# MetaHG/mitsuba2

Hardware: AMD Instinct MI355X
Metric: Msample/s, cbox 1024x1024@256spp per GPU, path integrator (max_depth=-1, rr_depth=5) (higher is better)
Workload: dtype f32

## Files before the change

mitsuba2_amd/csrc/device_scene.h:

```cpp
#pragma once
#include "device_math.h"
#include "device_bsdf.h"
#include "device_envmap.h"
#include "flat_worklist.h"

namespace mtsamd {

constexpr uint32_t kLeafFlag = 0x80000000u;
constexpr uint32_t kLeafCountShift = 27;
constexpr uint32_t kLeafStartMask = (1u << kLeafCountShift) - 1u;
constexpr uint32_t kNoPrim = 0xffffffffu;

#ifndef MTS_BVH4
#define MTS_BVH4 1
#endif
#if MTS_BVH4
typedef uint2 StackEntry;
typedef uint64_t StackRaw;
#else
typedef uint32_t StackEntry;
typedef uint32_t StackRaw;
#endif


// ... 20 lines not shown
    const float4 *nodes;
    const uint4 *qnodes;
    const uint4 *wnodes;
    uint32_t wroot, n_wnodes;
    float q_lo[3], q_step[3], q_inv_step[3];
    const float4 *tris;
    uint32_t root;
    uint32_t n_nodes, n_slots, n_prims;
    uint32_t lds_nodes;
    uint32_t lds_slots;
    uint32_t stack_depth;
    uint32_t walk_lds_depth, walk_blocks;
    StackEntry *walk_spill;
    const float *tri_pos;
    const float *tri_nrm;
    const float *tri_uv;
    const uint32_t *prim_shape;
    const DevShape *shapes;
    const DevBsdf *bsdfs;
    const DevEmitter *emitters; uint32_t n_emitters;
    uint32_t n_shapes, n_bsdfs;
    const DevTexture *textures; uint32_t n_textures;
    const float *area_pmf, *area_cdf;
    const float4 *flat_recs;
    const float4 *flat_pairs;
    uint32_t flat, n_pairs, n_clusters;
    int32_t env_emitter;
    const DevEnvmap *envmap;
    uint32_t general;
};
constexpr uint32_t kFlatMaxPrims = 64;

struct LdsView {
    const float4 *nodes;
    const float4 *tris;
    uint32_t *stack;
    uint32_t stride;
    StackEntry *spill;
    uint32_t spill_stride, stack_lds_depth;
    const float4 *flat;
    const float4 *pairs;
    const float4 *clusters;
    const DevShape *shapes;
    const DevBsdf *bsdfs;
    const DevEmitter *emitters;
    const float *pmf, *cdf;
    uint32_t *wl;
};

#ifndef MTS_FLAT_WORKLIST
#define MTS_FLAT_WORKLIST 1
#endif
#ifndef MTS_FLAT_WL_ROUNDS
#define MTS_FLAT_WL_ROUNDS 5
#endif
constexpr uint32_t kWlItems = 64u * MTS_FLAT_WL_ROUNDS;
constexpr uint32_t kWlWords = 128u + kWlItems / 2u;

inline uint32_t flat_shape_count(const SceneView &sv) { return sv.n_shapes; }

template <bool FLAT>
MTS_DEV LdsView lds_stage(const SceneView &sv, float4 *smem) {
    LdsView l = {};
    l.stride = blockDim.x;
    if (FLAT) {
        float4 *f = smem;
        for (uint32_t i = threadIdx.x; i < 4u * sv.n_prims; i += blockDim.x) f[i] = sv.flat_recs[i];
        l.flat = f;
        float4 *pr = f + 4u * sv.n_prims;
        for (uint32_t i = threadIdx.x; i < 5u * sv.n_pairs; i += blockDim.x) pr[i] = sv.flat_pairs[i];
        if (threadIdx.x < 5u) pr[5u * sv.n_pairs + threadIdx.x] = make_float4(0.0f, 0.0f, 0.0f, 0.0f);
        l.pairs = pr;
        float4 *cl = pr + 5u * sv.n_pairs + 5u;
        for (uint32_t i = threadIdx.x; i < 2u * sv.n_clusters; i += blockDim.x) cl[i] = sv.flat_pairs[5u * sv.n_pairs + i];
        l.clusters = cl;
        uint32_t *w = reinterpret_cast<uint32_t *>(cl + 2u * sv.n_clusters);
        const uint32_t n_sh = (sizeof(DevShape) / 4u) * sv.n_shapes, n_bs = (sizeof(DevBsdf) / 4u) * sv.n_bsdfs,
                       n_em = (sizeof(DevEmitter) / 4u) * sv.n_emitters;
        const uint32_t *g_sh = reinterpret_cast<const uint32_t *>(sv.shapes), *g_bs = reinterpret_cast<const uint32_t *>(sv.bsdfs),
                       *g_em = reinterpret_cast<const uint32_t *>(sv.emitters);
        for (uint32_t i = threadIdx.x; i < n_sh; i += blockDim.x) w[i] = g_sh[i];
        l.shapes = reinterpret_cast<const DevShape *>(w); w += n_sh;
        for (uint32_t i = threadIdx.x; i < n_bs; i += blockDim.x) w[i] = g_bs[i];
        l.bsdfs = reinterpret_cast<const DevBsdf *>(w); w += n_bs;
        for (uint32_t i = threadIdx.x; i < n_em; i += blockDim.x) w[i] = g_em[i];
        l.emitters = reinterpret_cast<const DevEmitter *>(w); w += n_em;
        float *fw = reinterpret_cast<float *>(w);
        for (uint32_t i = threadIdx.x; i < sv.n_prims; i += blockDim.x) { fw[i] = sv.area_pmf[i]; fw[sv.n_prims + i] = sv.area_cdf[i]; }
        l.pmf = fw; l.cdf = fw + sv.n_prims;
        const uint32_t wl_off = (uint32_t) (reinterpret_cast<uint32_t *>(fw + 2u * sv.n_prims) - reinterpret_cast<uint32_t *>(smem));
        l.wl = MTS_FLAT_WORKLIST ? reinterpret_cast<uint32_t *>(smem) + ((wl_off + 1u) & ~1u) : nullptr;
    } else {
        float4 *n = smem;
        float4 *t = n + 4u * sv.lds_nodes;
        for (uint32_t i = threadIdx.x; i < 4u * sv.lds_nodes; i += blockDim.x) n[i] = sv.nodes[i];
        for (uint32_t i = threadIdx.x; i < 3u * sv.lds_slots; i += blockDim.x) t[i] = sv.tris[i];
        l.nodes = n; l.tris = t;
        l.stack = reinterpret_cast<uint32_t *>(t + 3u * sv.lds_slots);
    }
    __syncthreads();
    return l;
}
inline size_t lds_bytes(const SceneView &sv, uint32_t block) {
    if (sv.flat)
        return (size_t) 64 * sv.n_prims + (size_t) 80 * (sv.n_pairs + 1) + (size_t) 32 * sv.n_clusters + sizeof(DevShape) * sv.n_shapes + sizeof(DevBsdf) * sv.n_bsdfs +
               sizeof(DevEmitter) * sv.n_emitters + (size_t) 8 * sv.n_prims +
               (MTS_FLAT_WORKLIST ? 4u + (size_t) 4 * kWlWords * (block / 64u) : 0u);
// ... 570 lines not shown
    bool any = false;
    if (!(MTS_CULL_STATS & 2)) tri_tests += sv.n_prims;
    const v2f ox = splat(o.x), oy = splat(o.y), oz = splat(o.z), dx = splat(d.x), dy = splat(d.y), dz = splat(d.z);
    const f3 inv = mk3(clamp_inv(d.x), clamp_inv(d.y), clamp_inv(d.z));
    const float4 *rec = lds.pairs;
    for (uint32_t c = 0; c < sv.n_clusters; ++c) {
        const float4 lo = lds.clusters[2u * c], hi = lds.clusters[2u * c + 1u];
        const uint32_t n = __float_as_uint(lo.w);
        const float ax = (lo.x - o.x) * inv.x, bx = (hi.x - o.x) * inv.x;
        const float ay = (lo.y - o.y) * inv.y, by = (hi.y - o.y) * inv.y;
        const float az = (lo.z - o.z) * inv.z, bz = (hi.z - o.z) * inv.z;
        const float tn = fmaxf(fmaxf(fminf(ax, bx), fminf(ay, by)), fmaxf(fminf(az, bz), mint));
        const float tf = fminf(fminf(fmaxf(ax, bx), fmaxf(ay, by)), fminf(fmaxf(az, bz), maxt));
        if (__ballot(!any && tn <= tf) == 0ull) { rec += 5u * n; continue; }
        if (MTS_CULL_STATS & 2) tri_tests += 2u * n;
        for (uint32_t i = 0; i < n; ++i) {
            const float4 q0 = rec[0], q1 = rec[1], q2 = rec[2], q3 = rec[3], q4 = rec[4];
            rec += 5;
            const PairUvt r = pair_test(q0, q1, q2, q3, q4, ox, oy, oz, dx, dy, dz);
            const bool ok_a = tri_accept(r.u.x, r.v.x, r.uv.x, r.t.x, mint, maxt);
            const bool ok_b = tri_accept(r.u.y, r.v.y, r.uv.y, r.t.y, mint, maxt);
            any = any || ok_a || ok_b;
        }
    }
    return any;
}

static_assert(kFlatMaxPrims <= 64u, "a pair mask is 32 bits");
template <bool ANY>
MTS_DEV bool traverse_flat_worklist(const SceneView &sv, const LdsView &lds, f3 o, f3 d, float mint, float maxt, Hit &hit, uint32_t &tri_tests) {
    const uint64_t active = __ballot(1);
    const uint32_t n_act = (uint32_t) __popcll(active), lane = lane_id(), rank = mask_rank(active);
    const f3 inv = mk3(clamp_inv(d.x), clamp_inv(d.y), clamp_inv(d.z));
    uint32_t pairs = 0u, first = 0u;
    for (uint32_t c = 0; c < sv.n_clusters; ++c) {
        const float4 lo = lds.clusters[2u * c], hi = lds.clusters[2u * c + 1u];
        const uint32_t n = __float_as_uint(lo.w);
        const float ax = (lo.x - o.x) * inv.x, bx = (hi.x - o.x) * inv.x;
        const float ay = (lo.y - o.y) * inv.y, by = (hi.y - o.y) * inv.y;
        const float az = (lo.z - o.z) * inv.z, bz = (hi.z - o.z) * inv.z;
        const float tn = fmaxf(fmaxf(fminf(ax, bx), fminf(ay, by)), fmaxf(fminf(az, bz), mint));
        const float tf = fminf(fminf(fmaxf(ax, bx), fmaxf(ay, by)), fminf(fmaxf(az, bz), maxt));
        const uint32_t bits = (uint32_t) ((1ull << n) - 1ull) << first;
        pairs |= tn <= tf ? bits : 0u;
        first += n;
    }
    const uint32_t cnt = (uint32_t) __popc(pairs);
    uint32_t pos = 0u, total = 0u;
#pragma unroll
    for (uint32_t b = 0; b < 6u; ++b) {
        const uint64_t m = __ballot((cnt >> b) & 1u);
        pos += mask_rank(m) << b; total += (uint32_t) __popcll(m) << b;
    }
    if (total > kWlItems || total > MTS_FLAT_WL_ROUNDS * n_act) return traverse_flat<ANY>(sv, lds, o, d, mint, maxt, hit, tri_tests);
    constexpr bool kRealCount = (MTS_CULL_STATS & (ANY ? 2 : 1)) != 0;
    if (!kRealCount) tri_tests += sv.n_prims;
    uint32_t *ws = lds.wl + (threadIdx.x >> 6) * kWlWords;
    unsigned long long *key = reinterpret_cast<unsigned long long *>(ws);
    uint16_t *tbl = reinterpret_cast<uint16_t *>(ws + 128u);
    if (ANY) ws[lane] = 0u;
    else key[lane] = kWlNoKey;
    wl_push_items(tbl, pos, pairs, lane);
    __builtin_amdgcn_fence(__ATOMIC_RELEASE, "wavefront");
    __builtin_amdgcn_wave_barrier();
    __builtin_amdgcn_fence(__ATOMIC_ACQUIRE, "wavefront");
    for (uint32_t j0 = 0u; j0 < total; j0 += n_act) {
        const uint32_t j = j0 + rank;
        const uint32_t item = j < total ? (uint32_t) tbl[j] : wl_item(lane, sv.n_pairs);
        const uint32_t owner = wl_item_owner(item), pair = wl_item_pair(item);
        const int addr = (int) (owner << 2);
        const float rox = __int_as_float(__builtin_amdgcn_ds_bpermute(addr, __float_as_int(o.x)));
        const float roy = __int_as_float(__builtin_amdgcn_ds_bpermute(addr, __float_as_int(o.y)));
        const float roz = __int_as_float(__builtin_amdgcn_ds_bpermute(addr, __float_as_int(o.z)));
        const float rdx = __int_as_float(__builtin_amdgcn_ds_bpermute(addr, __float_as_int(d.x)));
        const float rdy = __int_as_float(__builtin_amdgcn_ds_bpermute(addr, __float_as_int(d.y)));
        const float rdz = __int_as_float(__builtin_amdgcn_ds_bpermute(addr, __float_as_int(d.z)));
        const float rmint = __int_as_float(__builtin_amdgcn_ds_bpermute(addr, __float_as_int(mint)));
        const float rmaxt = __int_as_float(__builtin_amdgcn_ds_bpermute(addr, __float_as_int(maxt)));
        const float4 *rec = lds.pairs + 5u * pair;
        const float4 q0 = rec[0], q1 = rec[1], q2 = rec[2], q3 = rec[3], q4 = rec[4];
        const PairUvt r = pair_test(q0, q1, q2, q3, q4, splat(rox), splat(roy), splat(roz), splat(rdx), splat(rdy), splat(rdz));
        const bool ok_a = tri_accept(r.u.x, r.v.x, r.uv.x, r.t.x, rmint, rmaxt);
        const bool ok_b = tri_accept(r.u.y, r.v.y, r.uv.y, r.t.y, rmint, rmaxt);
        if (kRealCount && j < total) tri_tests += 2u;
        if (ANY) {
            if (ok_a || ok_b) ws[owner] = 1u;
        } else if (ok_a || ok_b) {
            const uint64_t ka = ok_a ? wl_key(r.t.x, 2u * pair) : kWlNoKey, kb = ok_b ? wl_key(r.t.y, 2u * pair + 1u) : kWlNoKey;
            atomicMin(&key[owner], (unsigned long long) (ka < kb ? ka : kb));
        }
        if (ANY) {
            __builtin_amdgcn_fence(__ATOMIC_RELEASE, "wavefront");
            __builtin_amdgcn_wave_barrier();
            __builtin_amdgcn_fence(__ATOMIC_ACQUIRE, "wavefront");
            if (__ballot(ws[lane] == 0u && pos + cnt > j0 + n_act) == 0ull) break;
        }
    }
    __builtin_amdgcn_fence(__ATOMIC_RELEASE, "wavefront");
    __builtin_amdgcn_wave_barrier();
    __builtin_amdgcn_fence(__ATOMIC_ACQUIRE, "wavefront");
    if (ANY) return ws[lane] != 0u;
    const uint64_t k = key[lane];
    hit.t = maxt; hit.prim = kNoPrim; hit.u = 0.0f; hit.v = 0.0f;
    if (k == kWlNoKey) return false;
    hit.prim = wl_key_prim(k);
    hit.t = flat_hit_uv(lds, o, d, hit.prim, hit.u, hit.v);
    return true;
// ... 345 lines not shown
```

mitsuba2_amd/csrc/kernels.h:

```cpp
#pragma once
#include <hip/hip_runtime.h>
#include "device_scene.h"
#include "device_spectral.h"

namespace mtsamd {

struct PoolView {
    float4 *ray_o, *ray_d, *thr, *res;
    uint4 *rng;
    uint2 *misc;
    float *xi;
    float2 *aux;
    float4 *hit, *sh_o, *sh_d, *nee;
    uint32_t *sh_slot;
};

struct RowMap { int32_t row0, local_rows, tile_rows, part, count; };
MTS_DEV int32_t row_to_global(const RowMap &m, int32_t lr) {
    if (m.count <= 1) return m.row0 + lr;
    int32_t t = lr / m.tile_rows;
    return (t * m.count + m.part) * m.tile_rows + (lr - t * m.tile_rows);
}
MTS_DEV int32_t row_to_local(const RowMap &m, int32_t gr) {
    if (m.count <= 1) { int32_t lr = gr - m.row0; return (lr >= 0 && lr < m.local_rows) ? lr : -1; }
// ... 48 lines not shown
    if (k >= chains) return n;
    const uint32_t lo = ((uint32_t) ((uint64_t) n * k / chains) + kChainAlign - 1u) & ~(kChainAlign - 1u);
    return lo < n ? lo : n;
}
__host__ __device__ inline uint32_t chunk_owner(uint32_t wave, uint32_t n, uint32_t chains) {
    if (chains <= 1u) return wave;
    uint32_t s_min = n, k = 0u, lo_k = 0u, extra_before = 0u;
    for (uint32_t c = 0; c < chains; ++c) {
        const uint32_t lo = chain_first(c, n, chains), hi = chain_first(c + 1u, n, chains);
        s_min = hi - lo < s_min ? hi - lo : s_min;
        if (wave >= lo && wave < hi) { k = c; lo_k = lo; }
    }
    const uint32_t i = wave - lo_k;
    if (i < s_min) return i * chains + k;
    for (uint32_t c = 0; c < k; ++c) extra_before += chain_first(c + 1u, n, chains) - chain_first(c, n, chains) - s_min;
    return s_min * chains + extra_before + (i - s_min);
}

struct FilmParams {
    const float4 *out_rgba;
    const float2 *out_pos;
    float *film;
    FilterView filter;
    uint64_t first_ordinal, n_samples;
    uint32_t plane_pix0, plane_pixels;
    RowMap rows;
    int32_t spp, crop_x, crop_y, crop_w, crop_h;
    int32_t row0, row1;
    int32_t pass_lr0, pass_rows, tiles_x, tiles_y;
    int32_t tile_h;
    int32_t slices;
    float *partials;
};

struct AdjointParams {
    RenderParams rp;
    FilterView filter;
    uint64_t n_samples;
    const float *dimage;
    const float *film;
    float *grad_bsdf;
    float *grad_tex;
    float *grad_emitter;
    float *grad_env;
    int32_t pg_bsdf; DevBsdf pg_plus, pg_minus; float pg_inv_2h; float *grad_param;
};

struct RayStreams {
    const float *ox, *oy, *oz, *dx, *dy, *dz, *mint, *maxt;
    const uint8_t *active;
};

size_t bounce_lds_bytes(const SceneView &sv);
hipError_t launch_bounce(const RenderParams &p, hipStream_t s);
hipError_t launch_split_stage(const RenderParams &p, int stage, hipStream_t s);
uint32_t trace_lds_depth(const SceneView &sv);
uint32_t trace_top_nodes(const SceneView &sv);
uint32_t trace_group();
size_t trace_spill_words(const SceneView &sv, uint32_t n_waves);
hipError_t launch_direct(const RenderParams &p, uint64_t n, hipStream_t s);
hipError_t launch_adjoint(const AdjointParams &a, hipStream_t s);
hipError_t launch_adjoint_env(const AdjointParams &a, hipStream_t s);
hipError_t launch_adjoint_param(const AdjointParams &a, hipStream_t s);
hipError_t launch_finish(const RenderParams &p, uint64_t alive, hipStream_t s);
hipError_t launch_mega(const RenderParams &p, hipStream_t s);
hipError_t upload_spectral_tables(const float *x, const float *y, const float *z, const float *d65);
hipError_t launch_film_gather(const FilmParams &p, hipStream_t s);
hipError_t launch_film_tiles(const FilmParams &p, hipStream_t s);
bool film_tiles_supported(const FilterView &f);
void film_tile_grid(FilmParams &p);
size_t film_partial_floats(const FilmParams &p);
hipError_t launch_ray_intersect(const SceneView &sv, uint64_t n, const RayStreams &r, int mode, float *t,
                                uint32_t *prim, uint32_t *shape, float *u, float *v, float *si26,
                                hipStream_t s);
hipError_t launch_ray_test(const SceneView &sv, uint64_t n, const RayStreams &r, uint8_t *hit, hipStream_t s);
hipError_t launch_camera_rays(const CameraView &cam, uint64_t n, const float *sx, const float *sy, const float *apx, const float *apy, float *ox,
                              float *oy, float *oz, float *dx, float *dy, float *dz, float *mint, float *maxt,
                              hipStream_t s);
hipError_t launch_imageblock_put(const FilterView &f, int32_t w, int32_t h, int32_t ox, int32_t oy, int32_t ch,
                                 int32_t border, uint64_t n, const float *pos, const float *values, float *data,
                                 hipStream_t s);
hipError_t launch_put_block(const float *src, int32_t sw, int32_t sh, int32_t sox, int32_t soy, int32_t sb,
                            float *dst, int32_t dw, int32_t dh, int32_t dox, int32_t doy, int32_t db, int32_t ch,
                            hipStream_t s);
hipError_t launch_square_stream(float4 *rgba, uint64_t n, hipStream_t s);
hipError_t launch_moment_pack(const float *values5, const float *squares5, float *film11, uint64_t n_pixels, hipStream_t s);
hipError_t launch_roughplastic_tables(DevBsdf *bsdfs, uint32_t index, float *table, const float *gl, int res_t, int res_r, hipStream_t s);
hipError_t launch_film_develop(const float *xyzaw, uint64_t n, float *rgba, hipStream_t s);
hipError_t launch_libm_eval(int fn, uint64_t n, const float *x, const float *y, float *out, hipStream_t s);

}
```

mitsuba2_amd/csrc/kernels.hip:

```cpp
#include "kernels.h"

namespace mtsamd {

constexpr int kBlock = 256;

struct PathState {
    f3 o, d; float mint, maxt;
    f3 thr; float bs_pdf;
    f3 res; float eta;
    Pcg32 rng;
    uint32_t ordinal, depth, flags;
};

template <bool NT = false>
MTS_DEV void load_state(const PoolView &p, size_t i, PathState &s) {
    float4 a = ld_stream<NT>(p.ray_o + i), b = ld_stream<NT>(p.ray_d + i), c = ld_stream<NT>(p.thr + i), e = ld_stream<NT>(p.res + i);
    uint4 r = ld_stream<NT>(p.rng + i); uint2 m = ld_stream<NT>(p.misc + i);
    s.o = mk3(a.x, a.y, a.z); s.mint = a.w;
    s.d = mk3(b.x, b.y, b.z); s.maxt = b.w;
    s.thr = mk3(c.x, c.y, c.z); s.bs_pdf = c.w;
    s.res = mk3(e.x, e.y, e.z); s.eta = e.w;
    s.rng.state = (uint64_t) r.x | ((uint64_t) r.y << 32);
    s.rng.inc = (uint64_t) r.z | ((uint64_t) r.w << 32);
    s.ordinal = m.x; s.depth = m.y & 0xffffu; s.flags = m.y >> 16;
}
template <bool NT = false>
MTS_DEV void store_state(const PoolView &p, size_t i, const PathState &s) {
    st_stream<NT>(p.ray_o + i, make_float4(s.o.x, s.o.y, s.o.z, s.mint));
    st_stream<NT>(p.ray_d + i, make_float4(s.d.x, s.d.y, s.d.z, s.maxt));
    st_stream<NT>(p.thr + i, make_float4(s.thr.x, s.thr.y, s.thr.z, s.bs_pdf));
    p.res[i] = make_float4(s.res.x, s.res.y, s.res.z, s.eta);
    st_stream<NT>(p.rng + i, make_uint4((uint32_t) s.rng.state, (uint32_t) (s.rng.state >> 32), (uint32_t) s.rng.inc,
                                        (uint32_t) (s.rng.inc >> 32)));
    st_stream<NT>(p.misc + i, make_uint2(s.ordinal, (s.depth & 0xffffu) | (s.flags << 16)));
}

struct Counters { uint32_t closest, any, segments, tri_tests; };

struct VertexRec {
    f3 E, Nc, Tp, rho; float invq;
    f3 T; int32_t rr_channel;
    uint32_t texel; f2 w1; int32_t bsdf; uint32_t has_bsdf;
    float ew, nk; int32_t em_hit, em_nee;
};

struct Deferred {
    Hit hit; bool found;
    bool pending; f3 so, sd; float smint, smaxt; float nee[4];
};

constexpr uint32_t kFlagDelta = 4u;

struct EnvGradCtx { f3 delta; float *grad; };
MTS_DEV void env_grad_add(const DevEnvmap &e, float u, float v, f3 coeff, const EnvGradCtx &eg) {
    u *= (float) (e.w - 1); v *= (float) (e.h - 1);
    const uint32_t px = min((uint32_t) u, (uint32_t) (e.w - 2)), py = min((uint32_t) v, (uint32_t) (e.h - 2));
    const float w1x = u - (float) px, w1y = v - (float) py, w0x = 1.0f - w1x, w0y = 1.0f - w1y;
// ... 778 lines not shown
#pragma unroll
    for (int k = 0; k < 4; ++k)
        for (int off = 32; off > 0; off >>= 1) tot[k] += __shfl_xor(tot[k], off);
    if (lane_id() == 0) {
        unsigned long long *ws = reinterpret_cast<unsigned long long *>(P.wave_stats + 4u * (size_t) ((gid >> 6) % P.n_waves));
        for (int k = 0; k < 4; ++k) if (tot[k]) atomicAdd(ws + k, (unsigned long long) tot[k]);
    }
}

hipError_t launch_direct(const RenderParams &p, uint64_t n, hipStream_t s) {
    const uint32_t blocks = (uint32_t) ((n + kBlock - 1) / kBlock);
    const size_t lds = bounce_lds_bytes(p.sv);
    if (p.sv.general == 2u) {
        if (p.sv.flat) hipLaunchKernelGGL((k_direct<true, true, true>), dim3(blocks), dim3(kBlock), lds, s, p, n);
        else hipLaunchKernelGGL((k_direct<false, true, true>), dim3(blocks), dim3(kBlock), lds, s, p, n);
    } else if (p.sv.general) {
        if (p.sv.flat) hipLaunchKernelGGL((k_direct<true, true>), dim3(blocks), dim3(kBlock), lds, s, p, n);
        else hipLaunchKernelGGL((k_direct<false, true>), dim3(blocks), dim3(kBlock), lds, s, p, n);
    } else {
        if (p.sv.flat) hipLaunchKernelGGL((k_direct<true, false>), dim3(blocks), dim3(kBlock), lds, s, p, n);
        else hipLaunchKernelGGL((k_direct<false, false>), dim3(blocks), dim3(kBlock), lds, s, p, n);
    }
    return hipGetLastError();
}

constexpr uint32_t kFlagZombie = 2u;

template <bool GENERAL, bool FLAT>
MTS_DEV bool step_deferred(const RenderParams &P, const LdsView &lds, PathState &s, Counters &c, Deferred &df) {
    return bounce_step<FLAT, false, FLAT ? 2 : 1, GENERAL>(P, lds, s, c, nullptr, &df);
}
template <bool GENERAL, bool FLAT>
MTS_DEV bool step_deferred(const RenderParams &P, const LdsView &lds, PathStateS &s, Counters &c, Deferred &df) {
    return bounce_step_spectral<FLAT, FLAT ? 2 : 1, GENERAL>(P, lds, s, c, &df);
}
MTS_DEV void add_nee(PathState &s, const float (&nee)[4]) { s.res = mk3(s.res.x + nee[0], s.res.y + nee[1], s.res.z + nee[2]); }
MTS_DEV void add_nee(PathStateS &s, const float (&nee)[4]) {
#pragma unroll
    for (int k = 0; k < kWav; ++k) s.res.v[k] += nee[k];
}
MTS_DEV void finish_path(const RenderParams &P, const PathState &s) { store_result(P, s); }
MTS_DEV void finish_path(const RenderParams &P, const PathStateS &s) { store_result_spectral(P, s); }
MTS_DEV void start_path(const RenderParams &P, uint64_t ordinal, uint32_t lp, uint32_t j, PathState &s) { generate_path(P, ordinal, lp, j, s); }
MTS_DEV void start_path(const RenderParams &P, uint64_t ordinal, uint32_t lp, uint32_t j, PathStateS &s) { generate_path_spectral(P, ordinal, lp, j, s); }

#ifndef MTS_SHADE_WAVES_MIN
#define MTS_SHADE_WAVES_MIN 4
#endif
#ifndef MTS_SHADE_WAVES_MIN_RGB_DIFFUSE
#define MTS_SHADE_WAVES_MIN_RGB_DIFFUSE 5
#endif
template <typename State, bool GENERAL> struct ShadeWaves { static constexpr int kMin = MTS_SHADE_WAVES_MIN; };
template <> struct ShadeWaves<PathState, false> { static constexpr int kMin = MTS_SHADE_WAVES_MIN_RGB_DIFFUSE; };
constexpr uint32_t kShadowRing = 128u;
template <typename State> struct ShadowRing { float4 *o, *d, *nee; uint32_t *slot; };

template <typename State, bool GENERAL>
MTS_DEV void drain_shadow_ring(const RenderParams &P, const LdsView &lds, const ShadowRing<State> &q, uint32_t head, uint32_t count,
                               size_t base, Counters &c) {
    __builtin_amdgcn_fence(__ATOMIC_SEQ_CST, "workgroup");
    const uint32_t lane = lane_id();
    if (lane < count) {
        const uint32_t k = (head + lane) & (kShadowRing - 1u);
        const float4 o = q.o[k], d = q.d[k];
        Hit h;
        if (!traverse<true, true>(P.sv, lds, mk3(o.x, o.y, o.z), mk3(d.x, d.y, d.z), o.w, d.w, h, c.tri_tests)) {
            const size_t slot = base + q.slot[k];
            float4 r = P.out.res[slot];
            const float4 e = q.nee[k];
            r.x += e.x; r.y += e.y; r.z += e.z; r.w += e.w;
            P.out.res[slot] = r;
        }
    }
}

#ifndef MTS_NT_STREAMS
#define MTS_NT_STREAMS 3
#endif
#ifndef MTS_PRIMARY_SHADOW
#define MTS_PRIMARY_SHADOW 1
#endif
#ifndef MTS_SURV_ORDER
#define MTS_SURV_ORDER 1
#endif
template <typename State, bool GENERAL, bool FLAT, bool INLINE = false>
__global__ __launch_bounds__(kBlock) __attribute__((amdgpu_waves_per_eu(FLAT ? MTS_BOUNCE_WAVES : ShadeWaves<State, GENERAL>::kMin, FLAT ? MTS_BOUNCE_WAVES : 8)))
void k_shade(const RenderParams P) {
    static_assert(FLAT || !INLINE, "the in-kernel shadow queue is for LDS-resident scenes");
    constexpr bool kNT = !FLAT && (MTS_NT_STREAMS & 2) != 0;
    extern __shared__ float4 smem[];
    LdsView lds = {};
    const uint32_t gw = (FLAT && P.gather_w > 4u) ? P.gather_w : 4u;
    const uint32_t hw = threadIdx.x >> 6;
    const uint32_t wave = gw > 4u ? P.wave_first + blockIdx.x * gw + hw : P.wave_first + ((blockIdx.x * kBlock + threadIdx.x) >> 6);
    const uint32_t wave_last = P.wave_last ? P.wave_last : P.n_waves;
    __shared__ uint32_t s_cnt[kBlock / 64u], s_surv[kBlock / 64u];
    __shared__ uint32_t s_pre[FLAT ? 1025 : 1];
    if (FLAT && gw > 4u) {
        const uint32_t g0 = wave - hw;
        for (uint32_t k = threadIdx.x; k < gw; k += kBlock) s_pre[k + 1u] = (g0 + k < wave_last) ? P.count_in[g0 + k] : 0u;
        if (threadIdx.x == 0u) s_pre[0] = 0u;
        __syncthreads();
        if (hw == 0u) {
            const uint32_t per = (gw + 63u) / 64u, ln = lane_id();
            uint32_t local = 0u;
            for (uint32_t i = 0; i < per; ++i) { const uint32_t idx = ln * per + i; if (idx < gw) local += s_pre[idx + 1u]; }
            uint32_t incl = local;
            for (uint32_t off = 1u; off < 64u; off <<= 1) { const uint32_t v = __shfl_up(incl, off); if (ln >= off) incl += v; }
            uint32_t run = incl - local;
            for (uint32_t i = 0; i < per; ++i) { const uint32_t idx = ln * per + i; if (idx < gw) { run += s_pre[idx + 1u]; s_pre[idx + 1u] = run; } }
        }
        __syncthreads();
        if (s_pre[gw] == 0u) {
            for (uint32_t k = threadIdx.x; k < gw; k += kBlock) if (g0 + k < wave_last) P.count_out[g0 + k] = 0u;
            return;
        }
        lds = lds_stage<true>(P.sv, smem);
    } else if (FLAT) {
        const uint32_t n_own = wave < wave_last ? P.count_in[wave] : 0u;
        if (lane_id() == 0u) { s_cnt[threadIdx.x >> 6] = n_own; s_surv[threadIdx.x >> 6] = (wave < wave_last && MTS_SURV_ORDER) ? min(P.count_in[P.n_waves + wave], n_own) : 0u; }
        const bool work = wave < wave_last && (n_own > 0u || P.cursor[wave] < P.cursor_end[wave]);
        if (!__syncthreads_or(work ? 1 : 0)) {
            if (wave < wave_last && lane_id() == 0u) {
                P.count_out[wave] = 0u;
                if (!INLINE) P.count_shadow[wave] = 0u;
            }
            return;
        }
        lds = lds_stage<true>(P.sv, smem);
    }
    ShadowRing<State> ring = {};
    if (INLINE) {
        float4 *qb = smem + P.lds_queue_offset + (size_t) (threadIdx.x >> 6) * (kShadowRing * 13u / 4u);
        ring.o = qb; ring.d = qb + kShadowRing; ring.nee = qb + 2u * kShadowRing;
        ring.slot = reinterpret_cast<uint32_t *>(qb + 3u * kShadowRing);
    }
    if (wave >= wave_last) return;
    const uint32_t lane = lane_id();
    const size_t base = (size_t) wave * P.seg_cap;
    uint32_t n_out = 0;
    Counters c = { 0u, 0u, 0u, 0u };
    uint32_t n_sh = 0;
    uint32_t q_head = 0, q_count = 0;
    const uint32_t wg_wave0 = wave - (threadIdx.x >> 6);
    const uint32_t n_valid = FLAT ? min((uint32_t) (kBlock / 64u), wave_last - wg_wave0) : 1u;
    uint32_t reg[2u * (kBlock / 64u)], surv4[kBlock / 64u], n_in = 0;
    if (FLAT && gw > 4u) {
        n_in = s_pre[gw];
    } else if (FLAT) {
#pragma unroll
        for (uint32_t g = 0; g < kBlock / 64u; ++g) {
            const uint32_t cg = g < n_valid ? s_cnt[g] : 0u;
            surv4[g] = g < n_valid ? s_surv[g] : 0u;
            reg[g] = surv4[g]; reg[kBlock / 64u + g] = cg - surv4[g];
            n_in += cg;
        }
    } else {
        n_in = __builtin_amdgcn_readfirstlane(P.count_in[wave]);
    }

    for (uint32_t i0 = FLAT ? 64u * (threadIdx.x >> 6) : 0u; i0 < n_in; i0 += 64u * n_valid) {
        State s;
        Deferred df;
        df.pending = false;
        bool alive = false, zombie_now = false;
        uint32_t depth0 = 0u;
        if (i0 + lane < n_in) {
            size_t i = base + i0 + lane;
            if (FLAT && gw > 4u) {
                const uint32_t idx = i0 + lane;
                uint32_t k = 0u;
                for (uint32_t step = gw >> 1; step; step >>= 1) if (s_pre[k + step] <= idx) k += step;
                i = (size_t) (wg_wave0 + k) * P.seg_cap + (idx - s_pre[k]);
            } else if (FLAT) {
                uint32_t r = 0u, j = i0 + lane;
#pragma unroll
                for (uint32_t g = 0; g + 1 < 2u * (kBlock / 64u); ++g)
                    if (r == g && j >= reg[g]) { j -= reg[g]; ++r; }
                constexpr uint32_t kW = kBlock / 64u;
                const uint32_t g = r >= kW ? r - kW : r;
                uint32_t off = 0u;
#pragma unroll
                for (uint32_t q = 0; q < kW; ++q) off = (r >= kW && g == q) ? surv4[q] : off;
                i = (size_t) (wg_wave0 + g) * P.seg_cap + off + j;
            }
            load_state<kNT>(P.in, i, s);
            if (s.flags & kFlagZombie) {
                finish_path(P, s);
            } else {
                depth0 = s.depth;
                if (!FLAT) {
                    const float4 h = ld_stream<kNT>(P.in.hit + i);
                    df.hit.t = h.x; df.hit.prim = __float_as_uint(h.y); df.hit.u = h.z; df.hit.v = h.w;
                    df.found = df.hit.prim != kNoPrim;
                }
                alive = step_deferred<GENERAL, FLAT>(P, lds, s, c, df);
                if (!alive) {
                    if (df.pending) { s.flags |= kFlagZombie; alive = true; zombie_now = true; }
                    else finish_path(P, s);
                }
            }
        }
        if (INLINE && MTS_FLAT_CULL && MTS_PRIMARY_SHADOW && P.sv.n_clusters > 1u && __ballot(depth0 != 1u && (i0 + lane < n_in)) == 0ull) {
            if (df.pending) {
                if (!traverse_flat_clustered_any(P.sv, lds, df.so, df.sd, df.smint, df.smaxt, c.tri_tests)) add_nee(s, df.nee);
                df.pending = false;
                if (zombie_now) { s.flags &= ~kFlagZombie; finish_path(P, s); alive = false; }
            }
        }
        const uint64_t m = __ballot(alive), ms = __ballot(alive && df.pending);
        if (alive) {
            const uint32_t slot = n_out + mask_rank(m);
            const size_t oidx = (FLAT && gw > 4u) ? ((size_t) wave + 4u * (slot / P.seg_cap)) * P.seg_cap + slot % P.seg_cap : base + slot;
            store_state<kNT>(P.out, oidx, s);
            if (df.pending) {
                if (INLINE) {
                    const uint32_t k = (q_head + q_count + mask_rank(ms)) & (kShadowRing - 1u);
                    ring.o[k] = make_float4(df.so.x, df.so.y, df.so.z, df.smint);
                    ring.d[k] = make_float4(df.sd.x, df.sd.y, df.sd.z, df.smaxt);
                    ring.nee[k] = make_float4(df.nee[0], df.nee[1], df.nee[2], df.nee[3]);
                    ring.slot[k] = (uint32_t) (oidx - base);
                } else {
                    const size_t q = base + n_sh + mask_rank(ms);
                    st_stream<kNT>(P.out.sh_o + q, make_float4(df.so.x, df.so.y, df.so.z, df.smint));
                    st_stream<kNT>(P.out.sh_d + q, make_float4(df.sd.x, df.sd.y, df.sd.z, df.smaxt));
                    st_stream<kNT>(P.out.nee + q, make_float4(df.nee[0], df.nee[1], df.nee[2], df.nee[3]));
                    st_stream<kNT>(P.out.sh_slot + q, slot);
                }
            }
        }
        n_out += (uint32_t) __popcll(m);
        n_sh += (uint32_t) __popcll(ms);
        if (INLINE) {
            q_count += (uint32_t) __popcll(ms);
            if (q_count >= 64u) {
                drain_shadow_ring<State, GENERAL>(P, lds, ring, q_head, 64u, base, c);
                q_head = (q_head + 64u) & (kShadowRing - 1u); q_count -= 64u;
            }
        }
    }
    if (INLINE && q_count > 0u) drain_shadow_ring<State, GENERAL>(P, lds, ring, q_head, q_count, base, c);

    const uint32_t n_surv = n_out;
    uint64_t cursor = P.cursor[wave];
    const uint64_t end = P.cursor_end[wave];
    while (n_out < P.target && cursor < end) {
        uint64_t left = end - cursor;
        uint32_t n_new = min(64u, P.target - n_out);
        if ((uint64_t) n_new > left) n_new = (uint32_t) left;
        if (lane < n_new) {
            State s;
            uint64_t ordinal; uint32_t lp, sj;
            cursor_sample(P, wave, cursor + lane, ordinal, lp, sj);
            start_path(P, ordinal, lp, sj, s);
            store_state<kNT>(P.out, base + n_out + lane, s);
        }
        n_out += n_new; cursor += n_new;
    }

    uint32_t tot[4] = { c.closest, c.any, c.segments, c.tri_tests };
#pragma unroll
    for (int k = 0; k < 4; ++k)
        for (int off = 32; off > 0; off >>= 1) tot[k] += __shfl_xor(tot[k], off);
    if (FLAT && gw > 4u) {
        for (uint32_t q = lane; q < gw / 4u; q += 64u) {
            const uint32_t w2 = wave + 4u * q, lo = q * P.seg_cap;
            if (w2 < wave_last) P.count_out[w2] = n_out > lo ? min(n_out - lo, P.seg_cap) : 0u;
        }
    }
    if (lane == 0) {
        if (!(FLAT && gw > 4u)) P.count_out[wave] = n_out;
        if (FLAT && !(gw > 4u)) P.count_out[P.n_waves + wave] = n_surv;
        if (!INLINE) P.count_shadow[wave] = n_sh;
        P.cursor[wave] = cursor;
// ... 310 lines not shown
                  (unsigned long long) tri_tests);
}

#if MTS_TRACE_PROF
extern "C" __attribute__((visibility("default"))) int mtsamd_debug_trace_prof(unsigned long long *out, int reset) {
    static unsigned long long host[64 * 64];
    if (hipMemcpyFromSymbol(host, HIP_SYMBOL(g_trace_prof), sizeof(host)) != hipSuccess) return -1;
    for (int i = 0; i < 64; ++i) { out[i] = 0; for (int c = 0; c < 64; ++c) out[i] += host[64 * c + i]; }
    if (reset) { for (auto &h : host) h = 0; if (hipMemcpyToSymbol(HIP_SYMBOL(g_trace_prof), host, sizeof(host)) != hipSuccess) return -1; }
    return 0;
}
#endif

uint32_t trace_top_nodes(const SceneView &sv) { return std::min(sv.n_wnodes, kTraceTopNodes); }
uint32_t trace_group() { return kTraceGroup; }
size_t trace_lds_bytes(const SceneView &sv) {
    return (size_t) 64 * trace_top_nodes(sv) + sizeof(StackEntry) * (std::min(sv.stack_depth, kTraceLdsDepth) + 1u) * kTraceBlock;
}
uint32_t trace_lds_depth(const SceneView &sv) { return std::min(sv.stack_depth, kTraceLdsDepth); }
size_t trace_spill_words(const SceneView &sv, uint32_t n_waves) {
    const uint32_t spill = sv.stack_depth > kTraceLdsDepth ? sv.stack_depth - kTraceLdsDepth : 0u;
    const uint32_t spill_f = sv.stack_depth > kFinishLdsDepth ? sv.stack_depth - kFinishLdsDepth : 0u;
    const size_t trace = (size_t) 2 * ((n_waves + kTraceGroup - 1) / kTraceGroup) * spill * kTraceBlock;
    const size_t finish = (size_t) n_waves * spill_f * 64u;
    return (sizeof(StackEntry) / 4) * std::max(trace, finish);
}
static hipError_t allow_lds(const void *fn, size_t bytes) {
    return bytes > 48u * 1024u ? hipFuncSetAttribute(fn, hipFuncAttributeMaxDynamicSharedMemorySize, (int) bytes) : hipSuccess;
}

hipError_t launch_split_stage(const RenderParams &p, int stage, hipStream_t s) {
    const uint32_t n_launch = (p.wave_last ? p.wave_last : p.n_waves) - p.wave_first;
    const uint32_t shade_blocks = (n_launch * 64u + kBlock - 1) / kBlock, trace_blocks = (n_launch + kTraceGroup - 1) / kTraceGroup;
    if (stage == 0) {
        if (hipError_t e = allow_lds(reinterpret_cast<const void *>(&k_trace<false, false>), trace_lds_bytes(p.sv))) return e;
        hipLaunchKernelGGL((k_trace<false, false>), dim3(trace_blocks), dim3(kTraceBlock), trace_lds_bytes(p.sv), s, p);
    } else if (stage == 1) {
        if (p.spectral && p.sv.general) hipLaunchKernelGGL((k_shade<PathStateS, true, false>), dim3(shade_blocks), dim3(kBlock), 0, s, p);
        else if (p.spectral) hipLaunchKernelGGL((k_shade<PathStateS, false, false>), dim3(shade_blocks), dim3(kBlock), 0, s, p);
        else if (p.sv.general) hipLaunchKernelGGL((k_shade<PathState, true, false>), dim3(shade_blocks), dim3(kBlock), 0, s, p);
        else hipLaunchKernelGGL((k_shade<PathState, false, false>), dim3(shade_blocks), dim3(kBlock), 0, s, p);
    } else {
        if (hipError_t e = allow_lds(reinterpret_cast<const void *>(&k_trace<true, false>), trace_lds_bytes(p.sv))) return e;
        hipLaunchKernelGGL((k_trace<true, false>), dim3(trace_blocks), dim3(kTraceBlock), trace_lds_bytes(p.sv), s, p);
    }
    return hipGetLastError();
}

hipError_t launch_bounce(const RenderParams &p_, hipStream_t s) {
    RenderParams p = p_;
    if (p.split == 3) {
        const uint32_t n_launch = (p.wave_last ? p.wave_last : p.n_waves) - p.wave_first;
        const uint32_t shade_blocks = p.gather_w > 4u ? (n_launch + p.gather_w - 1u) / p.gather_w : (n_launch * 64u + kBlock - 1) / kBlock;
        const size_t scene_bytes = (bounce_lds_bytes(p.sv) + 15u) & ~(size_t) 15u;
        p.lds_queue_offset = (uint32_t) (scene_bytes / 16u);
        const size_t lds = scene_bytes + (size_t) (kBlock / 64u) * kShadowRing * 52u;
        if (p.spectral && p.sv.general) hipLaunchKernelGGL((k_shade<PathStateS, true, true, true>), dim3(shade_blocks), dim3(kBlock), lds, s, p);
        else if (p.spectral) hipLaunchKernelGGL((k_shade<PathStateS, false, true, true>), dim3(shade_blocks), dim3(kBlock), lds, s, p);
        else if (p.sv.general) hipLaunchKernelGGL((k_shade<PathState, true, true, true>), dim3(shade_blocks), dim3(kBlock), lds, s, p);
        else hipLaunchKernelGGL((k_shade<PathState, false, true, true>), dim3(shade_blocks), dim3(kBlock), lds, s, p);
        return hipGetLastError();
    }
    if (p.split == 2) {
        const uint32_t shade_blocks = (p.n_waves * 64u + kBlock - 1) / kBlock;
        const size_t lds = bounce_lds_bytes(p.sv);
        if (p.spectral && p.sv.general) hipLaunchKernelGGL((k_shade<PathStateS, true, true>), dim3(shade_blocks), dim3(kBlock), lds, s, p);
        else if (p.spectral) hipLaunchKernelGGL((k_shade<PathStateS, false, true>), dim3(shade_blocks), dim3(kBlock), lds, s, p);
        else if (p.sv.general) hipLaunchKernelGGL((k_shade<PathState, true, true>), dim3(shade_blocks), dim3(kBlock), lds, s, p);
        else hipLaunchKernelGGL((k_shade<PathState, false, true>), dim3(shade_blocks), dim3(kBlock), lds, s, p);
        hipLaunchKernelGGL((k_trace<true, true>), dim3((p.n_waves + kFlatGroup - 1) / kFlatGroup), dim3(kBlock), lds, s, p);
        return hipGetLastError();
    }
    if (p.split) {
        hipError_t e = launch_split_stage(p, 0, s);
        if (e == hipSuccess) e = launch_split_stage(p, 1, s);
        if (e == hipSuccess) e = launch_split_stage(p, 2, s);
        return e;
    }
    uint32_t blocks = (p.n_waves * 64u + kBlock - 1) / kBlock;
    if (p.spectral) {
        if (p.sv.general == 2u) {
            if (p.sv.flat) hipLaunchKernelGGL((k_bounce_spectral<true, true, true>), dim3(blocks), dim3(kBlock), bounce_lds_bytes(p.sv), s, p);
            else hipLaunchKernelGGL((k_bounce_spectral<false, true, true>), dim3(blocks), dim3(kBlock), bounce_lds_bytes(p.sv), s, p);
        } else if (p.sv.general) {
            if (p.sv.flat) hipLaunchKernelGGL((k_bounce_spectral<true, true>), dim3(blocks), dim3(kBlock), bounce_lds_bytes(p.sv), s, p);
            else hipLaunchKernelGGL((k_bounce_spectral<false, true>), dim3(blocks), dim3(kBlock), bounce_lds_bytes(p.sv), s, p);
        } else {
            if (p.sv.flat) hipLaunchKernelGGL((k_bounce_spectral<true, false>), dim3(blocks), dim3(kBlock), bounce_lds_bytes(p.sv), s, p);
            else hipLaunchKernelGGL((k_bounce_spectral<false, false>), dim3(blocks), dim3(kBlock), bounce_lds_bytes(p.sv), s, p);
        }
        return hipGetLastError();
    }
    if (p.sv.general == 2u) {
        if (p.sv.flat) hipLaunchKernelGGL((k_bounce<true, true, true>), dim3(blocks), dim3(kBlock), bounce_lds_bytes(p.sv), s, p);
        else hipLaunchKernelGGL((k_bounce<false, true, true>), dim3(blocks), dim3(kBlock), bounce_lds_bytes(p.sv), s, p);
    } else if (p.sv.general) {
        if (p.sv.flat) hipLaunchKernelGGL((k_bounce<true, true>), dim3(blocks), dim3(kBlock), bounce_lds_bytes(p.sv), s, p);
        else hipLaunchKernelGGL((k_bounce<false, true>), dim3(blocks), dim3(kBlock), bounce_lds_bytes(p.sv), s, p);
    } else {
        if (p.sv.flat) hipLaunchKernelGGL((k_bounce<true, false>), dim3(blocks), dim3(kBlock), bounce_lds_bytes(p.sv), s, p);
        else hipLaunchKernelGGL((k_bounce<false, false>), dim3(blocks), dim3(kBlock), bounce_lds_bytes(p.sv), s, p);
    }
    return hipGetLastError();
}

MTS_DEV float cubic_filter(float x, float B, float C) {
    x = fabsf(x);
    const float x2 = x * x, x3 = x2 * x;
    const float result = (1.0f / 6.0f) * (x < 1.0f
// ... 871 lines not shown
```

Measured before the change: 3671.

## Shrink shade LDS: pack shadow slot into NEE.w, dynamic prefix array, more worklist rounds

For RGB path state, the shadow-ray ring now stores the output slot index in the w lane of the NEE float4 instead of a separate slot array, cutting ring size from 52 to 48 bytes per entry. The static 1025-entry prefix array becomes dynamically allocated LDS placed after the rings and sized only when gather width needs it. The flat worklist round count rises from 5 to 8 so fewer rays fall back to full flat traversal. A static_assert checks that four k_shade workgroups still fit per CU. The trade is that the larger worklist and the reshuffled LDS could lower occupancy.

```diff
diff --git a/mitsuba2_amd/csrc/device_scene.h b/mitsuba2_amd/csrc/device_scene.h
--- a/mitsuba2_amd/csrc/device_scene.h
+++ b/mitsuba2_amd/csrc/device_scene.h
@@ -96,7 +96,7 @@
 #define MTS_FLAT_WORKLIST 1
 #endif
 #ifndef MTS_FLAT_WL_ROUNDS
-#define MTS_FLAT_WL_ROUNDS 5
+#define MTS_FLAT_WL_ROUNDS 8
 #endif
 constexpr uint32_t kWlItems = 64u * MTS_FLAT_WL_ROUNDS;
 constexpr uint32_t kWlWords = 128u + kWlItems / 2u;
@@ -773,7 +773,9 @@
         const uint64_t m = __ballot((cnt >> b) & 1u);
         pos += mask_rank(m) << b; total += (uint32_t) __popcll(m) << b;
     }
-    if (total > kWlItems || total > MTS_FLAT_WL_ROUNDS * n_act) return traverse_flat<ANY>(sv, lds, o, d, mint, maxt, hit, tri_tests);
+    const bool fallback = total > kWlItems || total > MTS_FLAT_WL_ROUNDS * n_act;
+    if (MTS_CULL_STATS & 12) tri_tests += (rank == 0u && ((MTS_CULL_STATS & 8) || fallback)) ? 1u : 0u;
+    if (fallback) return traverse_flat<ANY>(sv, lds, o, d, mint, maxt, hit, tri_tests);
     constexpr bool kRealCount = (MTS_CULL_STATS & (ANY ? 2 : 1)) != 0;
     if (!kRealCount) tri_tests += sv.n_prims;
     uint32_t *ws = lds.wl + (threadIdx.x >> 6) * kWlWords;
diff --git a/mitsuba2_amd/csrc/kernels.h b/mitsuba2_amd/csrc/kernels.h
--- a/mitsuba2_amd/csrc/kernels.h
+++ b/mitsuba2_amd/csrc/kernels.h
@@ -124,6 +124,15 @@
 };
 
 size_t bounce_lds_bytes(const SceneView &sv);
+constexpr uint32_t kShadowRing = 128u;
+constexpr uint32_t kShadeWaves = 4u;
+inline size_t shadow_ring_bytes(bool spectral) { return (size_t) kShadowRing * (spectral ? 52u : 48u); }
+inline size_t shade_ring_offset(const SceneView &sv, uint32_t block) { return (lds_bytes(sv, block) + 15u) & ~(size_t) 15u; }
+inline size_t shade_ring_lds_bytes(const SceneView &sv, bool spectral, uint32_t gather_w) {
+    return shade_ring_offset(sv, 64u * kShadeWaves) + kShadeWaves * shadow_ring_bytes(spectral) + (gather_w > 4u ? 4u * ((size_t) gather_w + 1u) : 0u);
+}
+static_assert(kShadeWaves * (48u * kShadowRing + 4u * kWlWords) + 4u + 512u + 6144u <= 160u * 1024u / 4u,
+              "work lists + shadow rings no longer fit 4 k_shade workgroups per CU");
 hipError_t launch_bounce(const RenderParams &p, hipStream_t s);
 hipError_t launch_split_stage(const RenderParams &p, int stage, hipStream_t s);
 uint32_t trace_lds_depth(const SceneView &sv);
diff --git a/mitsuba2_amd/csrc/kernels.hip b/mitsuba2_amd/csrc/kernels.hip
--- a/mitsuba2_amd/csrc/kernels.hip
+++ b/mitsuba2_amd/csrc/kernels.hip
@@ -3,6 +3,7 @@
 namespace mtsamd {
 
 constexpr int kBlock = 256;
+static_assert(kBlock == 64 * (int) kShadeWaves, "k_shade LDS sizing (kernels.h)");
 
 struct PathState {
     f3 o, d; float mint, maxt;
@@ -887,8 +888,18 @@
 #endif
 template <typename State, bool GENERAL> struct ShadeWaves { static constexpr int kMin = MTS_SHADE_WAVES_MIN; };
 template <> struct ShadeWaves<PathState, false> { static constexpr int kMin = MTS_SHADE_WAVES_MIN_RGB_DIFFUSE; };
-constexpr uint32_t kShadowRing = 128u;
-template <typename State> struct ShadowRing { float4 *o, *d, *nee; uint32_t *slot; };
+template <typename State> struct ShadowRing {
+    static constexpr bool kSlotInNee = false;
+    static constexpr uint32_t kFloat4 = kShadowRing * 13u / 4u;
+    float4 *o, *d, *nee; uint32_t *slot;
+};
+template <> struct ShadowRing<PathState> {
+    static constexpr bool kSlotInNee = true;
+    static constexpr uint32_t kFloat4 = kShadowRing * 3u;
+    float4 *o, *d, *nee; uint32_t *slot;
+};
+static_assert(ShadowRing<PathState>::kFloat4 * 16u == 48u * kShadowRing && ShadowRing<PathStateS>::kFloat4 * 16u == 52u * kShadowRing,
+              "ring sizes of shadow_ring_bytes()");
 
 template <typename State, bool GENERAL>
 MTS_DEV void drain_shadow_ring(const RenderParams &P, const LdsView &lds, const ShadowRing<State> &q, uint32_t head, uint32_t count,
@@ -900,10 +911,11 @@
         const float4 o = q.o[k], d = q.d[k];
         Hit h;
         if (!traverse<true, true>(P.sv, lds, mk3(o.x, o.y, o.z), mk3(d.x, d.y, d.z), o.w, d.w, h, c.tri_tests)) {
-            const size_t slot = base + q.slot[k];
+            const float4 e = q.nee[k];
+            const size_t slot = base + (ShadowRing<State>::kSlotInNee ? __float_as_uint(e.w) : q.slot[k]);
             float4 r = P.out.res[slot];
-            const float4 e = q.nee[k];
-            r.x += e.x; r.y += e.y; r.z += e.z; r.w += e.w;
+            r.x += e.x; r.y += e.y; r.z += e.z;
+            if (!ShadowRing<State>::kSlotInNee) r.w += e.w;
             P.out.res[slot] = r;
         }
     }
@@ -925,12 +937,12 @@
     constexpr bool kNT = !FLAT && (MTS_NT_STREAMS & 2) != 0;
     extern __shared__ float4 smem[];
     LdsView lds = {};
-    const uint32_t gw = (FLAT && P.gather_w > 4u) ? P.gather_w : 4u;
+    const uint32_t gw = (INLINE && P.gather_w > 4u) ? P.gather_w : 4u;
     const uint32_t hw = threadIdx.x >> 6;
     const uint32_t wave = gw > 4u ? P.wave_first + blockIdx.x * gw + hw : P.wave_first + ((blockIdx.x * kBlock + threadIdx.x) >> 6);
     const uint32_t wave_last = P.wave_last ? P.wave_last : P.n_waves;
     __shared__ uint32_t s_cnt[kBlock / 64u], s_surv[kBlock / 64u];
-    __shared__ uint32_t s_pre[FLAT ? 1025 : 1];
+    uint32_t *const s_pre = reinterpret_cast<uint32_t *>(smem + P.lds_queue_offset + kShadeWaves * ShadowRing<State>::kFloat4);
     if (FLAT && gw > 4u) {
         const uint32_t g0 = wave - hw;
         for (uint32_t k = threadIdx.x; k < gw; k += kBlock) s_pre[k + 1u] = (g0 + k < wave_last) ? P.count_in[g0 + k] : 0u;
@@ -966,9 +978,9 @@
     }
     ShadowRing<State> ring = {};
     if (INLINE) {
-        float4 *qb = smem + P.lds_queue_offset + (size_t) (threadIdx.x >> 6) * (kShadowRing * 13u / 4u);
+        float4 *qb = smem + P.lds_queue_offset + (size_t) (threadIdx.x >> 6) * ShadowRing<State>::kFloat4;
         ring.o = qb; ring.d = qb + kShadowRing; ring.nee = qb + 2u * kShadowRing;
-        ring.slot = reinterpret_cast<uint32_t *>(qb + 3u * kShadowRing);
+        ring.slot = ShadowRing<State>::kSlotInNee ? nullptr : reinterpret_cast<uint32_t *>(qb + 3u * kShadowRing);
     }
     if (wave >= wave_last) return;
     const uint32_t lane = lane_id();
@@ -1053,8 +1065,13 @@
                     const uint32_t k = (q_head + q_count + mask_rank(ms)) & (kShadowRing - 1u);
                     ring.o[k] = make_float4(df.so.x, df.so.y, df.so.z, df.smint);
                     ring.d[k] = make_float4(df.sd.x, df.sd.y, df.sd.z, df.smaxt);
-                    ring.nee[k] = make_float4(df.nee[0], df.nee[1], df.nee[2], df.nee[3]);
-                    ring.slot[k] = (uint32_t) (oidx - base);
+                    const uint32_t rslot = (uint32_t) (oidx - base);
+                    if (ShadowRing<State>::kSlotInNee) {
+                        ring.nee[k] = make_float4(df.nee[0], df.nee[1], df.nee[2], __uint_as_float(rslot));
+                    } else {
+                        ring.nee[k] = make_float4(df.nee[0], df.nee[1], df.nee[2], df.nee[3]);
+                        ring.slot[k] = rslot;
+                    }
                 } else {
                     const size_t q = base + n_sh + mask_rank(ms);
                     st_stream<kNT>(P.out.sh_o + q, make_float4(df.so.x, df.so.y, df.so.z, df.smint));
@@ -1471,9 +1488,8 @@
     if (p.split == 3) {
         const uint32_t n_launch = (p.wave_last ? p.wave_last : p.n_waves) - p.wave_first;
         const uint32_t shade_blocks = p.gather_w > 4u ? (n_launch + p.gather_w - 1u) / p.gather_w : (n_launch * 64u + kBlock - 1) / kBlock;
-        const size_t scene_bytes = (bounce_lds_bytes(p.sv) + 15u) & ~(size_t) 15u;
-        p.lds_queue_offset = (uint32_t) (scene_bytes / 16u);
-        const size_t lds = scene_bytes + (size_t) (kBlock / 64u) * kShadowRing * 52u;
+        p.lds_queue_offset = (uint32_t) (shade_ring_offset(p.sv, kBlock) / 16u);
+        const size_t lds = shade_ring_lds_bytes(p.sv, p.spectral != 0, p.gather_w);
         if (p.spectral && p.sv.general) hipLaunchKernelGGL((k_shade<PathStateS, true, true, true>), dim3(shade_blocks), dim3(kBlock), lds, s, p);
         else if (p.spectral) hipLaunchKernelGGL((k_shade<PathStateS, false, true, true>), dim3(shade_blocks), dim3(kBlock), lds, s, p);
         else if (p.sv.general) hipLaunchKernelGGL((k_shade<PathState, true, true, true>), dim3(shade_blocks), dim3(kBlock), lds, s, p);
```

After: 3797, median of 6. 1.03x the previous value.
